# microsoft/AI2BMD

Measured on NVIDIA H100. Metric: MD steps/sec, higher is better.
Workload: dtype f32

## Files before the change

ai2bmd_b200/csrc/k_edge_tc.cuh:

```cuda
#pragma once
#include "k_edge.cuh"
#include "tc_common.cuh"

namespace vb {

constexpr int TC_TE = 128;
constexpr int TC_STAGES = 2;
constexpr int TC_MAX_STAGES = 3;
constexpr int TC_SLABS = D / tc::SLAB_K;
static_assert((TC_SLABS & (TC_SLABS - 1)) == 0, "tc_slab rotates the slab order with a mask: TC_SLABS must be a power of two");
constexpr int TC_MAXJOBS = 12;
constexpr int TC_LT = D + LDS_PAD;
typedef float TcRow[TC_LT];

struct TcJob {
    const float* img;
    int accumulate;
};

struct TcShared {
    alignas(1024) uint8_t ring[TC_STAGES][tc::STAGE_BYTES];
    alignas(16) float tile[TC_TE][TC_LT];
    alignas(16) float abuf[TC_TE][TC_LT];
    EdgeMeta<TC_TE> meta;
// ... 440 lines not shown
#pragma unroll
                        for (int u = 0; u < 2; u++) {
                            const int row = g0 + rb + u;
                            const float4 dd = sh.meta.d[row];
                            const float4 Pf = ld4(&sh.tile[row][col]) + bb;
                            const float4 fp = silu4(Pf);
                            const float4 a1 = tir[u][0] * dd.x + tir[u][1] * dd.y + tir[u][2] * dd.z;
                            const float4 a2 = ujr[u][0] * dd.x + ujr[u][1] * dd.y + ujr[u][2] * dd.z;
                            const float4 wdot = (tir[u][0] - a1 * dd.x) * (ujr[u][0] - a2 * dd.x) + (tir[u][1] - a1 * dd.y) * (ujr[u][1] - a2 * dd.y) +
                                                (tir[u][2] - a1 * dd.z) * (ujr[u][2] - a2 * dd.z);
                            if (rb + u < grpw && row < nvalid) {
                                st4(P1 + (size_t)(e0 + row) * 3 * D + 2 * D + col, Pf);
                                st4(Fout + (size_t)(e0 + row) * D + col, fin[u] + fp * wdot);
                            }
                        }
                    }
                    handoff_arrive(H_EU);
                }
                TC_TLG(7);
            }
            csync();
            TC_TL(18);
            const int cch = threadIdx.x & (D - 1), grp = threadIdx.x >> 7;
            float bnd[2][3] = {{0.f, 0.f, 0.f}, {0.f, 0.f, 0.f}};
            tc_fwd_s1(sh, ws, lw, VN, SP, sh.abuf, e0, nvalid, cch, grp, TC2_NGRP, bnd);
            TC_TL(19);
            tc_fwd_s2(sh, ws, lw, SP, sh.tile, e0, nvalid, cch, grp, TC2_NGRP, bnd);
            TC_TL(20);
        } else {
            const int cch = threadIdx.x & (D - 1), grp = threadIdx.x >> 7;
            const int rpw = (nvalid + TC2_CWARPS - 1) / TC2_CWARPS, r0 = warp * rpw;
            tc::mbar_wait(&sh.b_tile, tpar);
            csync();
            TC_TL(2);
            float Areg[RPW];
            tc2_mma(sh, ring, sh.abuf, acc, a.jobs[J_DK].accumulate, warp, lane, nvalid);
            TC_TL(4);
            tc2_acc_to(sh.tile, acc, warp, lane, nvalid);
            csync();
            {
                TC_TL(5);
                const float4 bb = ldg4(lw.b1 + col);
#pragma unroll
                for (int r = 0; r < RPW; r++) {
                    if (r >= rpw) break;
                    const int row = r0 + r;
                    const float4 qi = ldg4(QKV + (size_t)sh.meta.dst[row] * 3 * D + col);
                    const float4 kj = ldg4(QKV + (size_t)sh.meta.src[row] * 3 * D + D + col);
                    const float4 P = ld4(&sh.tile[row][col]) + bb;
                    const float av = quad_sum(hsum4(qi * kj * silu4(P)));
                    Areg[r] = silu_(av) * sh.meta.C[row];
                    if ((r < rpw && row < nvalid)) {
                        st4(P1 + (size_t)(e0 + row) * 3 * D + col, P);
                        if ((lane & 3) == 0) ATT[(size_t)(e0 + row) * H + (lane >> 2)] = av;
                    }
                }
            }
            TC_TL(6);
            tc2_mma(sh, ring, sh.abuf, acc, a.jobs[J_DV].accumulate, warp, lane, nvalid);
            TC_TL(7);
            csync();
            tc2_acc_to(sh.tile, acc, warp, lane, nvalid);
            csync();
            {
                TC_TL(8);
                const float4 bb = ldg4(lw.b1 + D + col);
#pragma unroll
                for (int r = 0; r < RPW; r++) {
                    if (r >= rpw) break;
                    const int row = r0 + r;
                    const float4 vj = ldg4(QKV + (size_t)sh.meta.src[row] * 3 * D + 2 * D + col);
                    const float4 P = ld4(&sh.tile[row][col]) + bb;
                    st4(&sh.tile[row][col], vj * silu4(P) * Areg[r]);
                    if ((r < rpw && row < nvalid)) st4(P1 + (size_t)(e0 + row) * 3 * D + D + col, P);
                }
            }
            csync();
            TC_TL(9);
            tc_fwd_xa(sh, ws, sh.tile, e0, nvalid, cch, grp, TC2_NGRP);
            TC_TL(10);
            if (upd) tc2_mma(sh, ring, sh.abuf, acc, a.jobs[J_F].accumulate, warp, lane, nvalid);
            tc2_tile_to_a(sh, nvalid);
            TC_TL(11);
            if (upd) {
                csync();
                tc2_acc_to(sh.tile, acc, warp, lane, nvalid);
                csync();
                const float4 bb = ldg4(lw.b1 + 2 * D + col);
#pragma unroll 1
                for (int rb = 0; rb < RPW; rb += 2) {
                    if (rb >= rpw) break;
                    float4 tir[2][3], ujr[2][3], fin[2];
#pragma unroll
                    for (int u = 0; u < 2; u++) {
                        const int row = r0 + rb + u;
                        const size_t i3 = (size_t)sh.meta.dst[row] * 3, j3 = (size_t)sh.meta.src[row] * 3;
                        if (rb + u < rpw && row < nvalid) fin[u] = ldg4(Fin + (size_t)(e0 + row) * D + col);
                        else fin[u] = f4s(0.f);
#pragma unroll
                        for (int s = 0; s < 3; s++) {
                            tir[u][s] = ldg4(TU + (i3 + s) * 2 * D + col);
                            ujr[u][s] = ldg4(TU + (j3 + s) * 2 * D + D + col);
                        }
                    }
#pragma unroll
                    for (int u = 0; u < 2; u++) {
                        const int row = r0 + rb + u;
                        const float4 dd = sh.meta.d[row];
                        const float4 Pf = ld4(&sh.tile[row][col]) + bb;
                        const float4 fp = silu4(Pf);
                        const float4 a1 = tir[u][0] * dd.x + tir[u][1] * dd.y + tir[u][2] * dd.z;
                        const float4 a2 = ujr[u][0] * dd.x + ujr[u][1] * dd.y + ujr[u][2] * dd.z;
                        const float4 wdot = (tir[u][0] - a1 * dd.x) * (ujr[u][0] - a2 * dd.x) + (tir[u][1] - a1 * dd.y) * (ujr[u][1] - a2 * dd.y) +
                                            (tir[u][2] - a1 * dd.z) * (ujr[u][2] - a2 * dd.z);
                        if ((rb + u < rpw && row < nvalid)) {
                            st4(P1 + (size_t)(e0 + row) * 3 * D + 2 * D + col, Pf);
                            st4(Fout + (size_t)(e0 + row) * D + col, fin[u] + fp * wdot);
                        }
                    }
                }
            }
            TC_TL(12);
            float bnd[2][3] = {{0.f, 0.f, 0.f}, {0.f, 0.f, 0.f}};
            tc2_mma(sh, ring, sh.abuf, acc, a.jobs[J_S1].accumulate, warp, lane, nvalid);
            TC_TL(13);
            csync();
            tc2_acc_to(sh.tile, acc, warp, lane, nvalid);
            csync();
            TC_TL(14);
            tc_fwd_s1(sh, ws, lw, VN, SP, sh.tile, e0, nvalid, cch, grp, TC2_NGRP, bnd);
            TC_TL(15);
            if (threadIdx.x == 0 && it + 1 < my_tiles) {
                const int en = ((int)blockIdx.x + (it + 1) * (int)gridDim.x) * trows;
                tc::tma_prefetch_l2(Fin + (size_t)en * D, (uint32_t)min(trows, E - en) * D * 4);
            }
            tc2_mma(sh, ring, sh.abuf, acc, a.jobs[J_S2].accumulate, warp, lane, nvalid);
            TC_TL(16);
            csync();
            tc2_acc_to(sh.tile, acc, warp, lane, nvalid);
            csync();
            TC_TL(17);
            tc_fwd_s2(sh, ws, lw, SP, sh.tile, e0, nvalid, cch, grp, TC2_NGRP, bnd);
            TC_TL(18);
        }
        csync();
    }
    if (a.tl != nullptr && blockIdx.x == 0 && threadIdx.x == 0) a.tl[31] = (unsigned long long)clock64();
}

}

namespace vb {

template <int ROWS>
__global__ void __launch_bounds__(TC2_THREADS, 1) edge_bwd_tc_kernel(const __grid_constant__ EdgeTcArgs a) {
    pdl_entry();
    extern __shared__ __align__(1024) uint8_t dyn_raw[];
    TcShared& sh = *tc_shared_base(dyn_raw);
    const Workspace& ws = a.ws;
    const int l = a.layer;
    const bool upd = (l < L - 1);
    const int J_G3A = 0, J_G3B = 1, J_G4DV = 2, J_G4DK = 3, J_G4F = 4;
    const int J_LAST = upd ? J_G4F : J_G4DK;
    constexpr int RPW = ROWS / TC2_CWARPS;
    constexpr int RB4 = (RPW % 4 == 0) ? 4 : 2;
    constexpr bool SMALL = ROWS <= 64;
    constexpr int RBM = SMALL ? 2 : RB4;
    const int warp = threadIdx.x >> 5, lane = threadIdx.x & 31, col = lane * 4, hd = lane >> 2;
    const int E = ws.rowptr[ws.N];
    const int trows = min(ROWS, max(16, a.tile_rows));
    const int ntiles_total = (E + trows - 1) / trows;
    const int my_tiles = ((int)blockIdx.x < ntiles_total) ? (ntiles_total - (int)blockIdx.x + (int)gridDim.x - 1) / (int)gridDim.x : 0;
    if (a.tl != nullptr && blockIdx.x == 0 && threadIdx.x == 0) a.tl[0] = (unsigned long long)clock64();
    TcRing<ROWS> ring;
    tc2_setup(sh, ring, a.jobs, a.njobs, my_tiles);
    if (a.tl != nullptr && blockIdx.x == 0 && threadIdx.x == 0) a.tl[1] = (unsigned long long)clock64();

    float acc[32];
    const float* __restrict__ QKV = ws.QKV[l];
    const float* __restrict__ VN = ws.VN[l];
    const float* __restrict__ TU = ws.TU[l];
    const float* __restrict__ P1 = ws.P1[l];
    const float* __restrict__ SP = ws.SP[l];
    const float* __restrict__ ATT = ws.ATT[l];
    const int cch = threadIdx.x & (D - 1), grp = threadIdx.x >> 7;
    for (int it = 0; it < my_tiles; it++) {
        const int e0 = ((int)blockIdx.x + it * (int)gridDim.x) * trows;
        const int nvalid = min(trows, E - e0);
        const int rpw = (nvalid + TC2_CWARPS - 1) / TC2_CWARPS, r0 = warp * rpw;
        load_edge_meta<TC_TE, TC2_CTHREADS>(sh.meta, ws, e0, nvalid);
        csync();
        TC_TL(2);
        if constexpr (SMALL) {
#pragma unroll 1
            for (int rb = 0; rb < RPW; rb += RB4) {
                if (rb >= rpw) break;
                float4 sp[RB4][2], gM[RB4][3], vn[RB4][3];
#pragma unroll
                for (int u = 0; u < RB4; u++) {
                    const int row = r0 + rb + u;
                    const size_t e = (size_t)(e0 + ((rb + u < rpw && row < nvalid) ? row : 0));
                    const size_t i3 = (size_t)sh.meta.dst[row] * 3, j3 = (size_t)sh.meta.src[row] * 3;
                    sp[u][0] = ldg4(SP + e * 2 * D + col);
                    sp[u][1] = ldg4(SP + e * 2 * D + D + col);
#pragma unroll
                    for (int s = 0; s < 3; s++) { gM[u][s] = ldg4(ws.GVEC + (i3 + s) * D + col); vn[u][s] = ldg4(VN + (j3 + s) * D + col); }
                }
#pragma unroll
                for (int u = 0; u < RB4; u++) {
                    const int row = r0 + rb + u;
                    const bool mine = rb + u < rpw, ok = (mine && row < nvalid);
                    const size_t j3 = (size_t)sh.meta.src[row] * 3;
                    const float4 dd = sh.meta.d[row];
                    const float4 s1 = silu4(sp[u][0]), s2 = silu4(sp[u][1]);
                    const float4 gs1 = gM[u][0] * vn[u][0] + gM[u][1] * vn[u][1] + gM[u][2] * vn[u][2];
                    const float gx_ = warp_sum(hsum4(gM[u][0] * s2)), gy_ = warp_sum(hsum4(gM[u][1] * s2)), gz_ = warp_sum(hsum4(gM[u][2] * s2));
                    if (mine) {
                        st4(&sh.abuf[row][col], ok ? gs1 * dsilu4(sp[u][0]) : f4s(0.f));
                        st4(&sh.tile[row][col], ok ? (gM[u][0] * dd.x + gM[u][1] * dd.y + gM[u][2] * dd.z) * dsilu4(sp[u][1]) : f4s(0.f));
                        if (lane == 0) { sh.eacc[row][1] = gx_; sh.eacc[row][2] = gy_; sh.eacc[row][3] = gz_; }
                    }
                    if (ok) {
                        red4(ws.GVNMSG + (j3 + 0) * D + col, gM[u][0] * s1);
                        red4(ws.GVNMSG + (j3 + 1) * D + col, gM[u][1] * s1);
                        red4(ws.GVNMSG + (j3 + 2) * D + col, gM[u][2] * s1);
                    }
                }
            }
            TC_TL(3);
        } else {
#pragma unroll 1
            for (int rb = 0; rb < RPW; rb += RB4) {
                if (rb >= rpw) break;
                float4 sp[RB4], gM[RB4][3], vn[RB4][3];
#pragma unroll
                for (int u = 0; u < RB4; u++) {
                    const int row = r0 + rb + u;
                    const size_t e = (size_t)(e0 + ((rb + u < rpw && row < nvalid) ? row : 0));
                    const size_t i3 = (size_t)sh.meta.dst[row] * 3, j3 = (size_t)sh.meta.src[row] * 3;
                    sp[u] = ldg4(SP + e * 2 * D + col);
#pragma unroll
                    for (int s = 0; s < 3; s++) { gM[u][s] = ldg4(ws.GVEC + (i3 + s) * D + col); vn[u][s] = ldg4(VN + (j3 + s) * D + col); }
                }
#pragma unroll
                for (int u = 0; u < RB4; u++) {
                    const int row = r0 + rb + u;
                    const bool ok = (rb + u < rpw && row < nvalid);
                    const size_t j3 = (size_t)sh.meta.src[row] * 3;
                    const float4 s1 = silu4(sp[u]);
                    const float4 gs1 = gM[u][0] * vn[u][0] + gM[u][1] * vn[u][1] + gM[u][2] * vn[u][2];
                    if (rb + u < rpw) st4(&sh.abuf[row][col], ok ? gs1 * dsilu4(sp[u]) : f4s(0.f));
                    if (ok) {
                        red4(ws.GVNMSG + (j3 + 0) * D + col, gM[u][0] * s1);
                        red4(ws.GVNMSG + (j3 + 1) * D + col, gM[u][1] * s1);
                        red4(ws.GVNMSG + (j3 + 2) * D + col, gM[u][2] * s1);
                    }
                }
            }
            TC_TL(3);
#pragma unroll 4
            for (int r = 0; r < RPW; r++) {
                if (r >= rpw) break;
                const int row = r0 + r;
                const bool ok = (r < rpw && row < nvalid);
                const size_t e = (size_t)(e0 + (ok ? row : 0));
                const size_t i3 = (size_t)sh.meta.dst[row] * 3;
                const float4 dd = sh.meta.d[row];
                const float4 sp = ldg4(SP + e * 2 * D + D + col);
                const float4 s2 = silu4(sp);
                const float4 gM0 = ldg4(ws.GVEC + (i3 + 0) * D + col), gM1 = ldg4(ws.GVEC + (i3 + 1) * D + col),
                             gM2 = ldg4(ws.GVEC + (i3 + 2) * D + col);
                const float gx_ = warp_sum(hsum4(gM0 * s2)), gy_ = warp_sum(hsum4(gM1 * s2)), gz_ = warp_sum(hsum4(gM2 * s2));
                if (lane == 0) { sh.eacc[row][1] = gx_; sh.eacc[row][2] = gy_; sh.eacc[row][3] = gz_; }
                st4(&sh.tile[row][col], ok ? (gM0 * dd.x + gM1 * dd.y + gM2 * dd.z) * dsilu4(sp) : f4s(0.f));
            }
            TC_TL(5);
        }
        csync();
        tc2_mma(sh, ring, sh.abuf, acc, a.jobs[J_G3A].accumulate, warp, lane, nvalid);
        TC_TL(6);
        if constexpr (!SMALL) {
            tc2_tile_to_a(sh, nvalid);
            TC_TL(7);
        }
        tc2_mma(sh, ring, SMALL ? sh.tile : sh.abuf, acc, a.jobs[J_G3B].accumulate, warp, lane, nvalid);
        TC_TL(8);
        csync();
        tc2_acc_to(sh.tile, acc, warp, lane, nvalid);
        csync();
        TC_TL(9);
#pragma unroll 1
        for (int rb = 0; rb < RPW; rb += RBM) {
            if (rb >= rpw) break;
            float4 gxa[RBM], vjr[RBM], pdvr[RBM];
            float avr[RBM];
#pragma unroll
            for (int u = 0; u < RBM; u++) {
                const int row = r0 + rb + u;
                const size_t e = (size_t)(e0 + ((rb + u < rpw && row < nvalid) ? row : 0));
                gxa[u] = load_gxa(ws, (size_t)sh.meta.dst[row], col);
                vjr[u] = ldg4(QKV + (size_t)sh.meta.src[row] * 3 * D + 2 * D + col);
                pdvr[u] = ldg4(P1 + e * 3 * D + D + col);
                avr[u] = (rb + u < rpw && row < nvalid) ? __ldg(ATT + e * H + hd) : 0.f;
            }
#pragma unroll
            for (int u = 0; u < RBM; u++) {
                const int row = r0 + rb + u;
                const bool ok = (rb + u < rpw && row < nvalid);
                const size_t j = sh.meta.src[row];
                const float Ce = sh.meta.C[row];
                const float av = avr[u], sa = silu_(av), A = sa * Ce;
                const bool mine = rb + u < rpw;
                const float4 gm = mine ? ld4(&sh.tile[row][col]) + gxa[u] : f4s(0.f);
                const float4 dv = silu4(pdvr[u]);
                if (mine) st4(&sh.abuf[row][col], ok ? gm * vjr[u] * A * dsilu4(pdvr[u]) : f4s(0.f));
                const float gA = quad_sum(hsum4(gm * vjr[u] * dv));
                if (mine && (lane & 3) == 0) sh.gattn[row][hd] = gA * Ce * dsilu_(av);
                const float gc = warp_sum((lane & 3) == 0 ? gA * sa : 0.f);
                if (mine && lane == 0) sh.eacc[row][0] = gc;
                if (ok) red4(ws.GQKV + j * 3 * D + 2 * D + col, gm * dv * A);
            }
        }
        TC_TL(10);
        csync();
#pragma unroll 1
        for (int rb = 0; rb < RPW; rb += RB4) {
            if (rb >= rpw) break;
            float4 pdkr[RB4], qir[RB4], kjr[RB4];
#pragma unroll
            for (int u = 0; u < RB4; u++) {
                const int row = r0 + rb + u;
                const size_t e = (size_t)(e0 + ((rb + u < rpw && row < nvalid) ? row : 0));
                pdkr[u] = ldg4(P1 + e * 3 * D + col);
                qir[u] = ldg4(QKV + (size_t)sh.meta.dst[row] * 3 * D + col);
                kjr[u] = ldg4(QKV + (size_t)sh.meta.src[row] * 3 * D + D + col);
            }
#pragma unroll
            for (int u = 0; u < RB4; u++) {
                const int row = r0 + rb + u;
                const bool ok = (rb + u < rpw && row < nvalid);
                const size_t j = sh.meta.src[row];
                const float4 dk = silu4(pdkr[u]);
                const float gav = sh.gattn[row][hd];
                if (rb + u < rpw) st4(&sh.tile[row][col], ok ? qir[u] * kjr[u] * gav * dsilu4(pdkr[u]) : f4s(0.f));
                if (SMALL && rb + u < rpw) st4(&tc_aux(sh)[row][col], kjr[u] * dk * gav);
                if (ok) red4(ws.GQKV + j * 3 * D + D + col, qir[u] * dk * gav);
            }
        }
        TC_TL(12);
        csync();
        tc2_mma(sh, ring, sh.abuf, acc, a.jobs[J_G4DV].accumulate, warp, lane, nvalid);
        TC_TL(13);
        if constexpr (!SMALL) {
            tc2_tile_to_a(sh, nvalid);
            TC_TL(14);
            csync();
#pragma unroll 4
            for (int r = 0; r < RPW; r++) {
                if (r >= rpw) break;
                const int row = r0 + r;
                const size_t e = (size_t)(e0 + ((r < rpw && row < nvalid) ? row : 0));
                const float4 dk = silu4(ldg4(P1 + e * 3 * D + col));
                const float4 kj = ldg4(QKV + (size_t)sh.meta.src[row] * 3 * D + D + col);
                st4(&sh.tile[row][col], kj * dk * sh.gattn[row][hd]);
            }
            csync();
        }
        {
            const TcRow* const gqb = SMALL ? tc_aux(sh) : sh.tile;
            const int i_first = sh.meta.dst[0], i_last = sh.meta.dst[nvalid - 1];
            for (int i = i_first + grp; i <= i_last; i += TC2_NGRP) {
                const int q0 = ws.rowptr[i], q1 = ws.rowptr[i + 1];
                const int lo = max(q0, e0) - e0, hi = min(q1, e0 + nvalid) - e0;
                float gq = 0.f;
                for (int r = lo; r < hi; r++) gq += gqb[r][cch];
                if (q0 >= e0 && q1 <= e0 + nvalid) ws.GQKV[(size_t)i * 3 * D + cch] = gq;
                else atomicAdd(ws.GQKV + (size_t)i * 3 * D + cch, gq);
            }
        }
        TC_TL(15);
        if (upd) {
            TcRow* const gpfb = SMALL ? sh.abuf : sh.tile;
            csync();
#pragma unroll 1
            for (int rb = 0; rb < RPW; rb += 2) {
                if (rb >= rpw) break;
                float4 gfr[2], pfr[2], tir[2][3], ujr[2][3];
#pragma unroll
                for (int u = 0; u < 2; u++) {
                    const int row = r0 + rb + u;
                    const bool ok = (rb + u < rpw && row < nvalid);
                    const size_t e = (size_t)(e0 + (ok ? row : 0));
                    const size_t i3 = (size_t)sh.meta.dst[row] * 3, j3 = (size_t)sh.meta.src[row] * 3;
                    gfr[u] = ok ? ld4(ws.GF + e * D + col) : f4s(0.f);
                    pfr[u] = ldg4(P1 + e * 3 * D + 2 * D + col);
#pragma unroll
                    for (int s = 0; s < 3; s++) {
                        tir[u][s] = ldg4(TU + (i3 + s) * 2 * D + col);
                        ujr[u][s] = ldg4(TU + (j3 + s) * 2 * D + D + col);
                    }
                }
#pragma unroll
                for (int u = 0; u < 2; u++) {
                    const int row = r0 + rb + u;
                    const bool ok = (rb + u < rpw && row < nvalid);
                    const size_t e = (size_t)(e0 + (ok ? row : 0));
                    const size_t j3 = (size_t)sh.meta.src[row] * 3;
                    const float4 dd = sh.meta.d[row];
                    const float4 gfn = gfr[u], pf = pfr[u];
                    const float4 fp = silu4(pf);
                    const float dv3[3] = {dd.x, dd.y, dd.z};
                    const float4 a1 = tir[u][0] * dd.x + tir[u][1] * dd.y + tir[u][2] * dd.z;
                    const float4 a2 = ujr[u][0] * dd.x + ujr[u][1] * dd.y + ujr[u][2] * dd.z;
                    float4 w1[3], w2[3];
#pragma unroll
                    for (int s = 0; s < 3; s++) { w1[s] = tir[u][s] - a1 * dv3[s]; w2[s] = ujr[u][s] - a2 * dv3[s]; }
                    const float4 wdot = w1[0] * w2[0] + w1[1] * w2[1] + w1[2] * w2[2];
                    const float4 gwd = gfn * fp;
                    if (rb + u < rpw) {
                        st4(&gpfb[row][col], gfn * wdot * dsilu4(pf));
                        if (SMALL) st4(&tc_aux(sh)[row][col], gwd);
                    }
                    const float4 c1 = gwd * (w2[0] * dd.x + w2[1] * dd.y + w2[2] * dd.z);
                    const float4 c2 = gwd * (w1[0] * dd.x + w1[1] * dd.y + w1[2] * dd.z);
                    float gdl[3];
                    float4 gu[3];
#pragma unroll
                    for (int s = 0; s < 3; s++) {
                        const float4 gw1 = gwd * w2[s], gw2 = gwd * w1[s];
                        gu[s] = gw2 - c2 * dv3[s];
                        gdl[s] = warp_sum(hsum4(tir[u][s] * c1 + a1 * gw1 + ujr[u][s] * c2 + a2 * gw2));
                    }
                    if (lane == 0 && rb + u < rpw) { sh.eacc[row][1] -= gdl[0]; sh.eacc[row][2] -= gdl[1]; sh.eacc[row][3] -= gdl[2]; }
                    if (ok) {
                        red4(ws.GTU + (j3 + 0) * 2 * D + D + col, gu[0]);
                        red4(ws.GTU + (j3 + 1) * 2 * D + D + col, gu[1]);
                        red4(ws.GTU + (j3 + 2) * 2 * D + D + col, gu[2]);
                    }
                    (void)e;
                }
            }
            TC_TL(16);
            csync();
            tc2_mma(sh, ring, SMALL ? sh.tile : sh.abuf, acc, a.jobs[J_G4DK].accumulate, warp, lane, nvalid);
            TC_TL(17);
            if constexpr (!SMALL) {
                tc2_tile_to_a(sh, nvalid);
                TC_TL(18);
                csync();
#pragma unroll 4
                for (int r = 0; r < RPW; r++) {
                    if (r >= rpw) break;
                    const int row = r0 + r;
                    const bool ok = (r < rpw && row < nvalid);
                    const size_t e = (size_t)(e0 + (ok ? row : 0));
                    const float4 gfn = ok ? ld4(ws.GF + e * D + col) : f4s(0.f);
                    st4(&sh.tile[row][col], gfn * silu4(ldg4(P1 + e * 3 * D + 2 * D + col)));
                }
                csync();
            }
            {
                const TcRow* const gwb = SMALL ? tc_aux(sh) : sh.tile;
                const int i_first = sh.meta.dst[0], i_last = sh.meta.dst[nvalid - 1];
                for (int i = i_first + grp; i <= i_last; i += TC2_NGRP) {
                    const int q0 = ws.rowptr[i], q1 = ws.rowptr[i + 1];
                    const int lo = max(q0, e0) - e0, hi = min(q1, e0 + nvalid) - e0;
                    float gt0 = 0.f, gt1 = 0.f, gt2 = 0.f;
                    auto term = [&](int r, float u0, float u1, float u2) {
                        const float4 dd = sh.meta.d[r];
                        const float gw = gwb[r][cch];
                        const float a2 = u0 * dd.x + u1 * dd.y + u2 * dd.z;
                        const float w20 = u0 - a2 * dd.x, w21 = u1 - a2 * dd.y, w22 = u2 - a2 * dd.z;
                        const float wd = w20 * dd.x + w21 * dd.y + w22 * dd.z;
                        gt0 += gw * (w20 - wd * dd.x);
                        gt1 += gw * (w21 - wd * dd.y);
                        gt2 += gw * (w22 - wd * dd.z);
                    };
                    int r = lo;
                    for (; r + 4 <= hi; r += 4) {
                        float u[4][3];
#pragma unroll
                        for (int q = 0; q < 4; q++) {
                            const size_t j3 = (size_t)sh.meta.src[r + q] * 3;
                            u[q][0] = __ldg(TU + (j3 + 0) * 2 * D + D + cch);
                            u[q][1] = __ldg(TU + (j3 + 1) * 2 * D + D + cch);
                            u[q][2] = __ldg(TU + (j3 + 2) * 2 * D + D + cch);
                        }
#pragma unroll
                        for (int q = 0; q < 4; q++) term(r + q, u[q][0], u[q][1], u[q][2]);
                    }
                    for (; r < hi; r++) {
                        const size_t j3 = (size_t)sh.meta.src[r] * 3;
                        term(r, __ldg(TU + (j3 + 0) * 2 * D + D + cch), __ldg(TU + (j3 + 1) * 2 * D + D + cch),
                             __ldg(TU + (j3 + 2) * 2 * D + D + cch));
                    }
                    if (q0 >= e0 && q1 <= e0 + nvalid) {
                        ws.GTU[((size_t)i * 3 + 0) * 2 * D + cch] = gt0;
                        ws.GTU[((size_t)i * 3 + 1) * 2 * D + cch] = gt1;
                        ws.GTU[((size_t)i * 3 + 2) * 2 * D + cch] = gt2;
                    } else {
                        atomicAdd(ws.GTU + ((size_t)i * 3 + 0) * 2 * D + cch, gt0);
                        atomicAdd(ws.GTU + ((size_t)i * 3 + 1) * 2 * D + cch, gt1);
                        atomicAdd(ws.GTU + ((size_t)i * 3 + 2) * 2 * D + cch, gt2);
                    }
                }
            }
        }
        TC_TL(19);
        if (threadIdx.x < 3 && it + 1 < my_tiles) {
            const int en = ((int)blockIdx.x + (it + 1) * (int)gridDim.x) * trows;
            const uint32_t nn = (uint32_t)min(trows, E - en);
            if (threadIdx.x == 0) tc::tma_prefetch_l2(SP + (size_t)en * 2 * D, nn * 2 * D * 4);
            else if (threadIdx.x == 1) tc::tma_prefetch_l2(P1 + (size_t)en * 3 * D, nn * 3 * D * 4);
            else tc::tma_prefetch_l2(ATT + (size_t)en * H, nn * H * 4);
        }
        tc2_mma(sh, ring, (SMALL && !upd) ? sh.tile : sh.abuf, acc, a.jobs[J_LAST].accumulate, warp, lane, nvalid);
        TC_TL(20);
        if (!SMALL || !upd) csync();
        tc2_acc_to(sh.tile, acc, warp, lane, nvalid);
        csync();
        TC_TL(21);
#pragma unroll 4
        for (int r = 0; r < RPW; r++) {
            if (r >= rpw) break;
            const int row = r0 + r;
            if ((r < rpw && row < nvalid)) {
                float* g = ws.GF + (size_t)(e0 + row) * D + col;
                float4 v = ld4(&sh.tile[row][col]);
                if (upd) v = v + ld4(g);
                st4(g, v);
            }
        }
        if (threadIdx.x < nvalid) {
            float* ea = ws.eacc + (size_t)(e0 + threadIdx.x) * 4;
            st4(ea, ld4(ea) + ld4(&sh.eacc[threadIdx.x][0]));
        }
        TC_TL(22);
        csync();
    }
    if (a.tl != nullptr && blockIdx.x == 0 && threadIdx.x == 0) a.tl[31] = (unsigned long long)clock64();
}

}
```

Baseline: 1160.

## Warp-specialize small-tile edge backward to overlap MMA with elementwise gather work

```diff
diff --git a/ai2bmd_b200/csrc/k_edge_tc.cuh b/ai2bmd_b200/csrc/k_edge_tc.cuh
--- a/ai2bmd_b200/csrc/k_edge_tc.cuh
+++ b/ai2bmd_b200/csrc/k_edge_tc.cuh
@@ -616,6 +616,226 @@
 
 namespace vb {
 
+
+template <int RB, int MAXR>
+__device__ __forceinline__ void tc_bwd_gm_rows(TcShared& sh, const Workspace& ws, const float* __restrict__ QKV,
+                                               const float* __restrict__ P1, const float* __restrict__ ATT, const TcRow* gmb,
+                                               TcRow* pdvb, int e0, int nvalid, int r0, int rpw, int lane) {
+    const int col = lane * 4, hd = lane >> 2;
+#pragma unroll 1
+    for (int rb = 0; rb < MAXR; rb += RB) {
+        if (rb >= rpw) break;
+        float4 gxa[RB], vjr[RB], pdvr[RB];
+        float avr[RB];
+#pragma unroll
+        for (int u = 0; u < RB; u++) {
+            const int row = r0 + rb + u;
+            const size_t e = (size_t)(e0 + ((rb + u < rpw && row < nvalid) ? row : 0));
+            gxa[u] = load_gxa(ws, (size_t)sh.meta.dst[row], col);
+            vjr[u] = ldg4(QKV + (size_t)sh.meta.src[row] * 3 * D + 2 * D + col);
+            pdvr[u] = ldg4(P1 + e * 3 * D + D + col);
+            avr[u] = (rb + u < rpw && row < nvalid) ? __ldg(ATT + e * H + hd) : 0.f;
+        }
+#pragma unroll
+        for (int u = 0; u < RB; u++) {
+            const int row = r0 + rb + u;
+            const bool ok = (rb + u < rpw && row < nvalid);
+            const size_t j = sh.meta.src[row];
+            const float Ce = sh.meta.C[row];
+            const float av = avr[u], sa = silu_(av), A = sa * Ce;
+            const bool mine = rb + u < rpw;
+            const float4 gm = mine ? ld4(&gmb[row][col]) + gxa[u] : f4s(0.f);
+            const float4 dv = silu4(pdvr[u]);
+            if (mine) st4(&pdvb[row][col], ok ? gm * vjr[u] * A * dsilu4(pdvr[u]) : f4s(0.f));
+            const float gA = quad_sum(hsum4(gm * vjr[u] * dv));
+            if (mine && (lane & 3) == 0) sh.gattn[row][hd] = gA * Ce * dsilu_(av);
+            const float gc = warp_sum((lane & 3) == 0 ? gA * sa : 0.f);
+            if (mine && lane == 0) sh.eacc[row][0] = gc;
+            if (ok) red4(ws.GQKV + j * 3 * D + 2 * D + col, gm * dv * A);
+        }
+    }
+}
+
+template <int RB, int MAXR>
+__device__ __forceinline__ void tc_bwd_gpdk_rows(TcShared& sh, const Workspace& ws, const float* __restrict__ QKV,
+                                                 const float* __restrict__ P1, TcRow* pdkb, TcRow* gqb, int e0, int nvalid,
+                                                 int r0, int rpw, int lane) {
+    const int col = lane * 4, hd = lane >> 2;
+#pragma unroll 1
+    for (int rb = 0; rb < MAXR; rb += RB) {
+        if (rb >= rpw) break;
+        float4 pdkr[RB], qir[RB], kjr[RB];
+#pragma unroll
+        for (int u = 0; u < RB; u++) {
+            const int row = r0 + rb + u;
+            const size_t e = (size_t)(e0 + ((rb + u < rpw && row < nvalid) ? row : 0));
+            pdkr[u] = ldg4(P1 + e * 3 * D + col);
+            qir[u] = ldg4(QKV + (size_t)sh.meta.dst[row] * 3 * D + col);
+            kjr[u] = ldg4(QKV + (size_t)sh.meta.src[row] * 3 * D + D + col);
+        }
+#pragma unroll
+        for (int u = 0; u < RB; u++) {
+            const int row = r0 + rb + u;
+            const bool ok = (rb + u < rpw && row < nvalid);
+            const size_t j = sh.meta.src[row];
+            const float4 dk = silu4(pdkr[u]);
+            const float gav = sh.gattn[row][hd];
+            if (rb + u < rpw) st4(&pdkb[row][col], ok ? qir[u] * kjr[u] * gav * dsilu4(pdkr[u]) : f4s(0.f));
+            if (gqb != nullptr && rb + u < rpw) st4(&gqb[row][col], kjr[u] * dk * gav);
+            if (ok) red4(ws.GQKV + j * 3 * D + D + col, qir[u] * dk * gav);
+        }
+    }
+}
+
+template <int MAXR>
+__device__ __forceinline__ void tc_bwd_gq_rows(const TcShared& sh, const float* __restrict__ QKV, const float* __restrict__ P1,
+                                               TcRow* gqb, int e0, int nvalid, int r0, int rpw, int lane) {
+    const int col = lane * 4, hd = lane >> 2;
+#pragma unroll 4
+    for (int r = 0; r < MAXR; r++) {
+        if (r >= rpw) break;
+        const int row = r0 + r;
+        const size_t e = (size_t)(e0 + ((r < rpw && row < nvalid) ? row : 0));
+        const float4 dk = silu4(ldg4(P1 + e * 3 * D + col));
+        const float4 kj = ldg4(QKV + (size_t)sh.meta.src[row] * 3 * D + D + col);
+        st4(&gqb[row][col], kj * dk * sh.gattn[row][hd]);
+    }
+}
+
+template <int MAXR>
+__device__ __forceinline__ void tc_bwd_gpf_rows(TcShared& sh, const Workspace& ws, const float* __restrict__ P1,
+                                                const float* __restrict__ TU, TcRow* gpfb, int e0, int nvalid, int r0, int rpw,
+                                                int lane) {
+    const int col = lane * 4;
+#pragma unroll 1
+    for (int rb = 0; rb < MAXR; rb += 2) {
+        if (rb >= rpw) break;
+        float4 gfr[2], pfr[2], tir[2][3], ujr[2][3];
+#pragma unroll
+        for (int u = 0; u < 2; u++) {
+            const int row = r0 + rb + u;
+            const bool ok = (rb + u < rpw && row < nvalid);
+            const size_t e = (size_t)(e0 + (ok ? row : 0));
+            const size_t i3 = (size_t)sh.meta.dst[row] * 3, j3 = (size_t)sh.meta.src[row] * 3;
+            gfr[u] = ok ? ld4(ws.GF + e * D + col) : f4s(0.f);
+            pfr[u] = ldg4(P1 + e * 3 * D + 2 * D + col);
+#pragma unroll
+            for (int s = 0; s < 3; s++) {
+                tir[u][s] = ldg4(TU + (i3 + s) * 2 * D + col);
+                ujr[u][s] = ldg4(TU + (j3 + s) * 2 * D + D + col);
+            }
+        }
+#pragma unroll
+        for (int u = 0; u < 2; u++) {
+            const int row = r0 + rb + u;
+            const bool ok = (rb + u < rpw && row < nvalid);
+            const size_t j3 = (size_t)sh.meta.src[row] * 3;
+            const float4 dd = sh.meta.d[row];
+            const float4 gfn = gfr[u], pf = pfr[u];
+            const float4 fp = silu4(pf);
+            const float dv3[3] = {dd.x, dd.y, dd.z};
+            const float4 a1 = tir[u][0] * dd.x + tir[u][1] * dd.y + tir[u][2] * dd.z;
+            const float4 a2 = ujr[u][0] * dd.x + ujr[u][1] * dd.y + ujr[u][2] * dd.z;
+            float4 w1[3], w2[3];
+#pragma unroll
+            for (int s = 0; s < 3; s++) { w1[s] = tir[u][s] - a1 * dv3[s]; w2[s] = ujr[u][s] - a2 * dv3[s]; }
+            const float4 wdot = w1[0] * w2[0] + w1[1] * w2[1] + w1[2] * w2[2];
+            const float4 gwd = gfn * fp;
+            if (rb + u < rpw) st4(&gpfb[row][col], gfn * wdot * dsilu4(pf));
+            const float4 c1 = gwd * (w2[0] * dd.x + w2[1] * dd.y + w2[2] * dd.z);
+            const float4 c2 = gwd * (w1[0] * dd.x + w1[1] * dd.y + w1[2] * dd.z);
+            float gdl[3];
+            float4 gu[3];
+#pragma unroll
+            for (int s = 0; s < 3; s++) {
+                const float4 gw1 = gwd * w2[s], gw2 = gwd * w1[s];
+                gu[s] = gw2 - c2 * dv3[s];
+                gdl[s] = warp_sum(hsum4(tir[u][s] * c1 + a1 * gw1 + ujr[u][s] * c2 + a2 * gw2));
+            }
+            if (lane == 0 && rb + u < rpw) { sh.eacc[row][1] -= gdl[0]; sh.eacc[row][2] -= gdl[1]; sh.eacc[row][3] -= gdl[2]; }
+            if (ok) {
+                red4(ws.GTU + (j3 + 0) * 2 * D + D + col, gu[0]);
+                red4(ws.GTU + (j3 + 1) * 2 * D + D + col, gu[1]);
+                red4(ws.GTU + (j3 + 2) * 2 * D + D + col, gu[2]);
+            }
+        }
+    }
+}
+
+template <int MAXR>
+__device__ __forceinline__ void tc_bwd_gwdot_rows(const Workspace& ws, const float* __restrict__ P1, TcRow* gwb, int e0,
+                                                  int nvalid, int r0, int rpw, int lane) {
+    const int col = lane * 4;
+#pragma unroll 4
+    for (int r = 0; r < MAXR; r++) {
+        if (r >= rpw) break;
+        const int row = r0 + r;
+        const bool ok = (r < rpw && row < nvalid);
+        const size_t e = (size_t)(e0 + (ok ? row : 0));
+        const float4 gfn = ok ? ld4(ws.GF + e * D + col) : f4s(0.f);
+        st4(&gwb[row][col], gfn * silu4(ldg4(P1 + e * 3 * D + 2 * D + col)));
+    }
+}
+
+__device__ __forceinline__ void tc_bwd_gq_sums(const TcShared& sh, const Workspace& ws, const TcRow* gqb, int e0, int nvalid,
+                                               int c, int grp, int ngrp) {
+    const int i_first = sh.meta.dst[0], i_last = sh.meta.dst[nvalid - 1];
+    for (int i = i_first + grp; i <= i_last; i += ngrp) {
+        const int q0 = ws.rowptr[i], q1 = ws.rowptr[i + 1];
+        const int lo = max(q0, e0) - e0, hi = min(q1, e0 + nvalid) - e0;
+        float gq = 0.f;
+        for (int r = lo; r < hi; r++) gq += gqb[r][c];
+        if (q0 >= e0 && q1 <= e0 + nvalid) ws.GQKV[(size_t)i * 3 * D + c] = gq;
+        else atomicAdd(ws.GQKV + (size_t)i * 3 * D + c, gq);
+    }
+}
+__device__ __forceinline__ void tc_bwd_gwdot_sums(const TcShared& sh, const Workspace& ws, const float* __restrict__ TU,
+                                                  const TcRow* gwb, int e0, int nvalid, int c, int grp, int ngrp) {
+    const int i_first = sh.meta.dst[0], i_last = sh.meta.dst[nvalid - 1];
+    for (int i = i_first + grp; i <= i_last; i += ngrp) {
+        const int q0 = ws.rowptr[i], q1 = ws.rowptr[i + 1];
+        const int lo = max(q0, e0) - e0, hi = min(q1, e0 + nvalid) - e0;
+        float gt0 = 0.f, gt1 = 0.f, gt2 = 0.f;
+        auto term = [&](int r, float u0, float u1, float u2) {
+            const float4 dd = sh.meta.d[r];
+            const float gw = gwb[r][c];
+            const float a2 = u0 * dd.x + u1 * dd.y + u2 * dd.z;
+            const float w20 = u0 - a2 * dd.x, w21 = u1 - a2 * dd.y, w22 = u2 - a2 * dd.z;
+            const float wd = w20 * dd.x + w21 * dd.y + w22 * dd.z;
+            gt0 += gw * (w20 - wd * dd.x);
+            gt1 += gw * (w21 - wd * dd.y);
+            gt2 += gw * (w22 - wd * dd.z);
+        };
+        int r = lo;
+        for (; r + 4 <= hi; r += 4) {
+            float u[4][3];
+#pragma unroll
+            for (int q = 0; q < 4; q++) {
+                const size_t j3 = (size_t)sh.meta.src[r + q] * 3;
+                u[q][0] = __ldg(TU + (j3 + 0) * 2 * D + D + c);
+                u[q][1] = __ldg(TU + (j3 + 1) * 2 * D + D + c);
+                u[q][2] = __ldg(TU + (j3 + 2) * 2 * D + D + c);
+            }
+#pragma unroll
+            for (int q = 0; q < 4; q++) term(r + q, u[q][0], u[q][1], u[q][2]);
+        }
+        for (; r < hi; r++) {
+            const size_t j3 = (size_t)sh.meta.src[r] * 3;
+            term(r, __ldg(TU + (j3 + 0) * 2 * D + D + c), __ldg(TU + (j3 + 1) * 2 * D + D + c),
+                 __ldg(TU + (j3 + 2) * 2 * D + D + c));
+        }
+        if (q0 >= e0 && q1 <= e0 + nvalid) {
+            ws.GTU[((size_t)i * 3 + 0) * 2 * D + c] = gt0;
+            ws.GTU[((size_t)i * 3 + 1) * 2 * D + c] = gt1;
+            ws.GTU[((size_t)i * 3 + 2) * 2 * D + c] = gt2;
+        } else {
+            atomicAdd(ws.GTU + ((size_t)i * 3 + 0) * 2 * D + c, gt0);
+            atomicAdd(ws.GTU + ((size_t)i * 3 + 1) * 2 * D + c, gt1);
+            atomicAdd(ws.GTU + ((size_t)i * 3 + 2) * 2 * D + c, gt2);
+        }
+    }
+}
+
 template <int ROWS>
 __global__ void __launch_bounds__(TC2_THREADS, 1) edge_bwd_tc_kernel(const __grid_constant__ EdgeTcArgs a) {
     pdl_entry();
@@ -629,8 +849,7 @@
     constexpr int RPW = ROWS / TC2_CWARPS;
     constexpr int RB4 = (RPW % 4 == 0) ? 4 : 2;
     constexpr bool SMALL = ROWS <= 64;
-    constexpr int RBM = SMALL ? 2 : RB4;
-    const int warp = threadIdx.x >> 5, lane = threadIdx.x & 31, col = lane * 4, hd = lane >> 2;
+    const int warp = threadIdx.x >> 5, lane = threadIdx.x & 31, col = lane * 4;
     const int E = ws.rowptr[ws.N];
     const int trows = min(ROWS, max(16, a.tile_rows));
     const int ntiles_total = (E + trows - 1) / trows;
@@ -692,6 +911,67 @@
                 }
             }
             TC_TL(3);
+            enum : int { H_G4DV = 3 };
+            TcRow* const xb = tc_aux(sh);
+            constexpr int GRPW = ROWS / (TC2_CWARPS / 2);
+            const int gw = (warp >> 3) * 4 + (warp & 3), gt = gw * 32 + lane;
+            const int grpw = (nvalid + 7) / 8, g0 = gw * grpw;
+            const int gch = gt & (D - 1), ggrp = gt >> 7;
+            csync();
+            if (tc2_is_mma_warp(warp)) {
+                tc2_mma<ROWS, true>(sh, ring, sh.abuf, acc, a.jobs[J_G3A].accumulate, warp, lane, nvalid);
+                TC_TL(6);
+                tc2_mma<ROWS, true>(sh, ring, sh.tile, acc, a.jobs[J_G3B].accumulate, warp, lane, nvalid);
+                TC_TL(8);
+                tc2_acc_to(sh.abuf, acc, warp, lane, nvalid);
+            } else if (upd) {
+                tc_bwd_gpf_rows<GRPW>(sh, ws, P1, TU, xb, e0, nvalid, g0, grpw, lane);
+                TC_TLG(0);
+            }
+            csync();
+            TC_TL(9);
+            tc_bwd_gm_rows<2, RPW>(sh, ws, QKV, P1, ATT, sh.abuf, sh.abuf, e0, nvalid, r0, rpw, lane);
+            TC_TL(10);
+            __syncwarp();
+            tc_bwd_gpdk_rows<RB4, RPW>(sh, ws, QKV, P1, sh.tile, upd ? nullptr : xb, e0, nvalid, r0, rpw, lane);
+            csync();
+            TC_TL(12);
+            if (tc2_is_mma_warp(warp)) {
+                tc2_mma<ROWS, true>(sh, ring, sh.abuf, acc, a.jobs[J_G4DV].accumulate, warp, lane, nvalid);
+                if (upd) handoff_arrive(H_G4DV);
+                TC_TL(13);
+                if (upd) {
+                    tc2_mma<ROWS, true>(sh, ring, sh.tile, acc, a.jobs[J_G4DK].accumulate, warp, lane, nvalid);
+                    TC_TL(17);
+                }
+                if (threadIdx.x < 3 && it + 1 < my_tiles) {
+                    const int en = ((int)blockIdx.x + (it + 1) * (int)gridDim.x) * trows;
+                    const uint32_t nn = (uint32_t)min(trows, E - en);
+                    if (threadIdx.x == 0) tc::tma_prefetch_l2(SP + (size_t)en * 2 * D, nn * 2 * D * 4);
+                    else if (threadIdx.x == 1) tc::tma_prefetch_l2(P1 + (size_t)en * 3 * D, nn * 3 * D * 4);
+                    else tc::tma_prefetch_l2(ATT + (size_t)en * H, nn * H * 4);
+                }
+                tc2_mma<ROWS, true>(sh, ring, upd ? xb : sh.tile, acc, a.jobs[J_LAST].accumulate, warp, lane, nvalid);
+                TC_TL(20);
+            } else {
+                if (upd) {
+                    handoff_wait(H_G4DV);
+                    TC_TLG(4);
+                    tc_bwd_gq_rows<GRPW>(sh, QKV, P1, sh.abuf, e0, nvalid, g0, grpw, lane);
+                }
+                gather_sync();
+                tc_bwd_gq_sums(sh, ws, upd ? sh.abuf : xb, e0, nvalid, gch, ggrp, 2);
+                TC_TLG(5);
+                if (upd) {
+                    gather_sync();
+                    tc_bwd_gwdot_rows<GRPW>(ws, P1, sh.abuf, e0, nvalid, g0, grpw, lane);
+                    TC_TLG(6);
+                }
+            }
+            csync();
+            if (tc2_is_mma_warp(warp)) tc2_acc_to(sh.tile, acc, warp, lane, nvalid);
+            if (upd) tc_bwd_gwdot_sums(sh, ws, TU, sh.abuf, e0, nvalid, cch, grp, TC2_NGRP);
+            TC_TL(19);
         } else {
 #pragma unroll 1
             for (int rb = 0; rb < RPW; rb += RB4) {
@@ -739,249 +1019,59 @@
                 st4(&sh.tile[row][col], ok ? (gM0 * dd.x + gM1 * dd.y + gM2 * dd.z) * dsilu4(sp) : f4s(0.f));
             }
             TC_TL(5);
-        }
-        csync();
-        tc2_mma(sh, ring, sh.abuf, acc, a.jobs[J_G3A].accumulate, warp, lane, nvalid);
-        TC_TL(6);
-        if constexpr (!SMALL) {
+            csync();
+            tc2_mma(sh, ring, sh.abuf, acc, a.jobs[J_G3A].accumulate, warp, lane, nvalid);
+            TC_TL(6);
             tc2_tile_to_a(sh, nvalid);
             TC_TL(7);
-        }
-        tc2_mma(sh, ring, SMALL ? sh.tile : sh.abuf, acc, a.jobs[J_G3B].accumulate, warp, lane, nvalid);
-        TC_TL(8);
-        csync();
-        tc2_acc_to(sh.tile, acc, warp, lane, nvalid);
-        csync();
-        TC_TL(9);
-#pragma unroll 1
-        for (int rb = 0; rb < RPW; rb += RBM) {
-            if (rb >= rpw) break;
-            float4 gxa[RBM], vjr[RBM], pdvr[RBM];
-            float avr[RBM];
-#pragma unroll
-            for (int u = 0; u < RBM; u++) {
-                const int row = r0 + rb + u;
-                const size_t e = (size_t)(e0 + ((rb + u < rpw && row < nvalid) ? row : 0));
-                gxa[u] = load_gxa(ws, (size_t)sh.meta.dst[row], col);
-                vjr[u] = ldg4(QKV + (size_t)sh.meta.src[row] * 3 * D + 2 * D + col);
-                pdvr[u] = ldg4(P1 + e * 3 * D + D + col);
-                avr[u] = (rb + u < rpw && row < nvalid) ? __ldg(ATT + e * H + hd) : 0.f;
-            }
-#pragma unroll
-            for (int u = 0; u < RBM; u++) {
-                const int row = r0 + rb + u;
-                const bool ok = (rb + u < rpw && row < nvalid);
-                const size_t j = sh.meta.src[row];
-                const float Ce = sh.meta.C[row];
-                const float av = avr[u], sa = silu_(av), A = sa * Ce;
-                const bool mine = rb + u < rpw;
-                const float4 gm = mine ? ld4(&sh.tile[row][col]) + gxa[u] : f4s(0.f);
-                const float4 dv = silu4(pdvr[u]);
-                if (mine) st4(&sh.abuf[row][col], ok ? gm * vjr[u] * A * dsilu4(pdvr[u]) : f4s(0.f));
-                const float gA = quad_sum(hsum4(gm * vjr[u] * dv));
-                if (mine && (lane & 3) == 0) sh.gattn[row][hd] = gA * Ce * dsilu_(av);
-                const float gc = warp_sum((lane & 3) == 0 ? gA * sa : 0.f);
-                if (mine && lane == 0) sh.eacc[row][0] = gc;
-                if (ok) red4(ws.GQKV + j * 3 * D + 2 * D + col, gm * dv * A);
-            }
-        }
-        TC_TL(10);
-        csync();
-#pragma unroll 1
-        for (int rb = 0; rb < RPW; rb += RB4) {
-            if (rb >= rpw) break;
-            float4 pdkr[RB4], qir[RB4], kjr[RB4];
-#pragma unroll
-            for (int u = 0; u < RB4; u++) {
-                const int row = r0 + rb + u;
-                const size_t e = (size_t)(e0 + ((rb + u < rpw && row < nvalid) ? row : 0));
-                pdkr[u] = ldg4(P1 + e * 3 * D + col);
-                qir[u] = ldg4(QKV + (size_t)sh.meta.dst[row] * 3 * D + col);
-                kjr[u] = ldg4(QKV + (size_t)sh.meta.src[row] * 3 * D + D + col);
-            }
-#pragma unroll
-            for (int u = 0; u < RB4; u++) {
-                const int row = r0 + rb + u;
-                const bool ok = (rb + u < rpw && row < nvalid);
-                const size_t j = sh.meta.src[row];
-                const float4 dk = silu4(pdkr[u]);
-                const float gav = sh.gattn[row][hd];
-                if (rb + u < rpw) st4(&sh.tile[row][col], ok ? qir[u] * kjr[u] * gav * dsilu4(pdkr[u]) : f4s(0.f));
-                if (SMALL && rb + u < rpw) st4(&tc_aux(sh)[row][col], kjr[u] * dk * gav);
-                if (ok) red4(ws.GQKV + j * 3 * D + D + col, qir[u] * dk * gav);
-            }
-        }
-        TC_TL(12);
-        csync();
-        tc2_mma(sh, ring, sh.abuf, acc, a.jobs[J_G4DV].accumulate, warp, lane, nvalid);
-        TC_TL(13);
-        if constexpr (!SMALL) {
+            tc2_mma(sh, ring, sh.abuf, acc, a.jobs[J_G3B].accumulate, warp, lane, nvalid);
+            TC_TL(8);
+            csync();
+            tc2_acc_to(sh.tile, acc, warp, lane, nvalid);
+            csync();
+            TC_TL(9);
+            tc_bwd_gm_rows<RB4, RPW>(sh, ws, QKV, P1, ATT, sh.tile, sh.abuf, e0, nvalid, r0, rpw, lane);
+            TC_TL(10);
+            csync();
+            tc_bwd_gpdk_rows<RB4, RPW>(sh, ws, QKV, P1, sh.tile, nullptr, e0, nvalid, r0, rpw, lane);
+            TC_TL(12);
+            csync();
+            tc2_mma(sh, ring, sh.abuf, acc, a.jobs[J_G4DV].accumulate, warp, lane, nvalid);
+            TC_TL(13);
             tc2_tile_to_a(sh, nvalid);
             TC_TL(14);
             csync();
-#pragma unroll 4
-            for (int r = 0; r < RPW; r++) {
-                if (r >= rpw) break;
-                const int row = r0 + r;
-                const size_t e = (size_t)(e0 + ((r < rpw && row < nvalid) ? row : 0));
-                const float4 dk = silu4(ldg4(P1 + e * 3 * D + col));
-                const float4 kj = ldg4(QKV + (size_t)sh.meta.src[row] * 3 * D + D + col);
-                st4(&sh.tile[row][col], kj * dk * sh.gattn[row][hd]);
-            }
-            csync();
-        }
-        {
-            const TcRow* const gqb = SMALL ? tc_aux(sh) : sh.tile;
-            const int i_first = sh.meta.dst[0], i_last = sh.meta.dst[nvalid - 1];
-            for (int i = i_first + grp; i <= i_last; i += TC2_NGRP) {
-                const int q0 = ws.rowptr[i], q1 = ws.rowptr[i + 1];
-                const int lo = max(q0, e0) - e0, hi = min(q1, e0 + nvalid) - e0;
-                float gq = 0.f;
-                for (int r = lo; r < hi; r++) gq += gqb[r][cch];
-                if (q0 >= e0 && q1 <= e0 + nvalid) ws.GQKV[(size_t)i * 3 * D + cch] = gq;
-                else atomicAdd(ws.GQKV + (size_t)i * 3 * D + cch, gq);
-            }
-        }
-        TC_TL(15);
-        if (upd) {
-            TcRow* const gpfb = SMALL ? sh.abuf : sh.tile;
-            csync();
-#pragma unroll 1
-            for (int rb = 0; rb < RPW; rb += 2) {
-                if (rb >= rpw) break;
-                float4 gfr[2], pfr[2], tir[2][3], ujr[2][3];
-#pragma unroll
-                for (int u = 0; u < 2; u++) {
-                    const int row = r0 + rb + u;
-                    const bool ok = (rb + u < rpw && row < nvalid);
-                    const size_t e = (size_t)(e0 + (ok ? row : 0));
-                    const size_t i3 = (size_t)sh.meta.dst[row] * 3, j3 = (size_t)sh.meta.src[row] * 3;
-                    gfr[u] = ok ? ld4(ws.GF + e * D + col) : f4s(0.f);
-                    pfr[u] = ldg4(P1 + e * 3 * D + 2 * D + col);
-#pragma unroll
-                    for (int s = 0; s < 3; s++) {
-                        tir[u][s] = ldg4(TU + (i3 + s) * 2 * D + col);
-                        ujr[u][s] = ldg4(TU + (j3 + s) * 2 * D + D + col);
-                    }
-                }
-#pragma unroll
-                for (int u = 0; u < 2; u++) {
-                    const int row = r0 + rb + u;
-                    const bool ok = (rb + u < rpw && row < nvalid);
-                    const size_t e = (size_t)(e0 + (ok ? row : 0));
-                    const size_t j3 = (size_t)sh.meta.src[row] * 3;
-                    const float4 dd = sh.meta.d[row];
-                    const float4 gfn = gfr[u], pf = pfr[u];
-                    const float4 fp = silu4(pf);
-                    const float dv3[3] = {dd.x, dd.y, dd.z};
-                    const float4 a1 = tir[u][0] * dd.x + tir[u][1] * dd.y + tir[u][2] * dd.z;
-                    const float4 a2 = ujr[u][0] * dd.x + ujr[u][1] * dd.y + ujr[u][2] * dd.z;
-                    float4 w1[3], w2[3];
-#pragma unroll
-                    for (int s = 0; s < 3; s++) { w1[s] = tir[u][s] - a1 * dv3[s]; w2[s] = ujr[u][s] - a2 * dv3[s]; }
-                    const float4 wdot = w1[0] * w2[0] + w1[1] * w2[1] + w1[2] * w2[2];
-                    const float4 gwd = gfn * fp;
-                    if (rb + u < rpw) {
-                        st4(&gpfb[row][col], gfn * wdot * dsilu4(pf));
-                        if (SMALL) st4(&tc_aux(sh)[row][col], gwd);
-                    }
-                    const float4 c1 = gwd * (w2[0] * dd.x + w2[1] * dd.y + w2[2] * dd.z);
-                    const float4 c2 = gwd * (w1[0] * dd.x + w1[1] * dd.y + w1[2] * dd.z);
-                    float gdl[3];
-                    float4 gu[3];
-#pragma unroll
-                    for (int s = 0; s < 3; s++) {
-                        const float4 gw1 = gwd * w2[s], gw2 = gwd * w1[s];
-                        gu[s] = gw2 - c2 * dv3[s];
-                        gdl[s] = warp_sum(hsum4(tir[u][s] * c1 + a1 * gw1 + ujr[u][s] * c2 + a2 * gw2));
-                    }
-                    if (lane == 0 && rb + u < rpw) { sh.eacc[row][1] -= gdl[0]; sh.eacc[row][2] -= gdl[1]; sh.eacc[row][3] -= gdl[2]; }
-                    if (ok) {
-                        red4(ws.GTU + (j3 + 0) * 2 * D + D + col, gu[0]);
-                        red4(ws.GTU + (j3 + 1) * 2 * D + D + col, gu[1]);
-                        red4(ws.GTU + (j3 + 2) * 2 * D + D + col, gu[2]);
-                    }
-                    (void)e;
-                }
-            }
-            TC_TL(16);
-            csync();
-            tc2_mma(sh, ring, SMALL ? sh.tile : sh.abuf, acc, a.jobs[J_G4DK].accumulate, warp, lane, nvalid);
-            TC_TL(17);
-            if constexpr (!SMALL) {
+            tc_bwd_gq_rows<RPW>(sh, QKV, P1, sh.tile, e0, nvalid, r0, rpw, lane);
+            csync();
+            tc_bwd_gq_sums(sh, ws, sh.tile, e0, nvalid, cch, grp, TC2_NGRP);
+            TC_TL(15);
+            if (upd) {
+                csync();
+                tc_bwd_gpf_rows<RPW>(sh, ws, P1, TU, sh.tile, e0, nvalid, r0, rpw, lane);
+                TC_TL(16);
+                csync();
+                tc2_mma(sh, ring, sh.abuf, acc, a.jobs[J_G4DK].accumulate, warp, lane, nvalid);
+                TC_TL(17);
                 tc2_tile_to_a(sh, nvalid);
                 TC_TL(18);
                 csync();
-#pragma unroll 4
-                for (int r = 0; r < RPW; r++) {
-                    if (r >= rpw) break;
-                    const int row = r0 + r;
-                    const bool ok = (r < rpw && row < nvalid);
-                    const size_t e = (size_t)(e0 + (ok ? row : 0));
-                    const float4 gfn = ok ? ld4(ws.GF + e * D + col) : f4s(0.f);
-                    st4(&sh.tile[row][col], gfn * silu4(ldg4(P1 + e * 3 * D + 2 * D + col)));
-                }
+                tc_bwd_gwdot_rows<RPW>(ws, P1, sh.tile, e0, nvalid, r0, rpw, lane);
                 csync();
-            }
-            {
-                const TcRow* const gwb = SMALL ? tc_aux(sh) : sh.tile;
-                const int i_first = sh.meta.dst[0], i_last = sh.meta.dst[nvalid - 1];
-                for (int i = i_first + grp; i <= i_last; i += TC2_NGRP) {
-                    const int q0 = ws.rowptr[i], q1 = ws.rowptr[i + 1];
-                    const int lo = max(q0, e0) - e0, hi = min(q1, e0 + nvalid) - e0;
-                    float gt0 = 0.f, gt1 = 0.f, gt2 = 0.f;
-                    auto term = [&](int r, float u0, float u1, float u2) {
-                        const float4 dd = sh.meta.d[r];
-                        const float gw = gwb[r][cch];
-                        const float a2 = u0 * dd.x + u1 * dd.y + u2 * dd.z;
-                        const float w20 = u0 - a2 * dd.x, w21 = u1 - a2 * dd.y, w22 = u2 - a2 * dd.z;
-                        const float wd = w20 * dd.x + w21 * dd.y + w22 * dd.z;
-                        gt0 += gw * (w20 - wd * dd.x);
-                        gt1 += gw * (w21 - wd * dd.y);
-                        gt2 += gw * (w22 - wd * dd.z);
-                    };
-                    int r = lo;
-                    for (; r + 4 <= hi; r += 4) {
-                        float u[4][3];
-#pragma unroll
-                        for (int q = 0; q < 4; q++) {
-                            const size_t j3 = (size_t)sh.meta.src[r + q] * 3;
-                            u[q][0] = __ldg(TU + (j3 + 0) * 2 * D + D + cch);
-                            u[q][1] = __ldg(TU + (j3 + 1) * 2 * D + D + cch);
-                            u[q][2] = __ldg(TU + (j3 + 2) * 2 * D + D + cch);
-                        }
-#pragma unroll
-                        for (int q = 0; q < 4; q++) term(r + q, u[q][0], u[q][1], u[q][2]);
-                    }
-                    for (; r < hi; r++) {
-                        const size_t j3 = (size_t)sh.meta.src[r] * 3;
-                        term(r, __ldg(TU + (j3 + 0) * 2 * D + D + cch), __ldg(TU + (j3 + 1) * 2 * D + D + cch),
-                             __ldg(TU + (j3 + 2) * 2 * D + D + cch));
-                    }
-                    if (q0 >= e0 && q1 <= e0 + nvalid) {
-                        ws.GTU[((size_t)i * 3 + 0) * 2 * D + cch] = gt0;
-                        ws.GTU[((size_t)i * 3 + 1) * 2 * D + cch] = gt1;
-                        ws.GTU[((size_t)i * 3 + 2) * 2 * D + cch] = gt2;
-                    } else {
-                        atomicAdd(ws.GTU + ((size_t)i * 3 + 0) * 2 * D + cch, gt0);
-                        atomicAdd(ws.GTU + ((size_t)i * 3 + 1) * 2 * D + cch, gt1);
-                        atomicAdd(ws.GTU + ((size_t)i * 3 + 2) * 2 * D + cch, gt2);
-                    }
-                }
-            }
-        }
-        TC_TL(19);
-        if (threadIdx.x < 3 && it + 1 < my_tiles) {
-            const int en = ((int)blockIdx.x + (it + 1) * (int)gridDim.x) * trows;
-            const uint32_t nn = (uint32_t)min(trows, E - en);
-            if (threadIdx.x == 0) tc::tma_prefetch_l2(SP + (size_t)en * 2 * D, nn * 2 * D * 4);
-            else if (threadIdx.x == 1) tc::tma_prefetch_l2(P1 + (size_t)en * 3 * D, nn * 3 * D * 4);
-            else tc::tma_prefetch_l2(ATT + (size_t)en * H, nn * H * 4);
-        }
-        tc2_mma(sh, ring, (SMALL && !upd) ? sh.tile : sh.abuf, acc, a.jobs[J_LAST].accumulate, warp, lane, nvalid);
-        TC_TL(20);
-        if (!SMALL || !upd) csync();
-        tc2_acc_to(sh.tile, acc, warp, lane, nvalid);
+                tc_bwd_gwdot_sums(sh, ws, TU, sh.tile, e0, nvalid, cch, grp, TC2_NGRP);
+            }
+            TC_TL(19);
+            if (threadIdx.x < 3 && it + 1 < my_tiles) {
+                const int en = ((int)blockIdx.x + (it + 1) * (int)gridDim.x) * trows;
+                const uint32_t nn = (uint32_t)min(trows, E - en);
+                if (threadIdx.x == 0) tc::tma_prefetch_l2(SP + (size_t)en * 2 * D, nn * 2 * D * 4);
+                else if (threadIdx.x == 1) tc::tma_prefetch_l2(P1 + (size_t)en * 3 * D, nn * 3 * D * 4);
+                else tc::tma_prefetch_l2(ATT + (size_t)en * H, nn * H * 4);
+            }
+            tc2_mma(sh, ring, sh.abuf, acc, a.jobs[J_LAST].accumulate, warp, lane, nvalid);
+            TC_TL(20);
+            csync();
+            tc2_acc_to(sh.tile, acc, warp, lane, nvalid);
+        }
         csync();
         TC_TL(21);
 #pragma unroll 4
```

Result: faster. 1176 (median of 6 runs) (+1.4%).
